# jsh58/Genrich

Measured on AMD Instinct MI355X. Metric: genome bases p-scored/sec, hg38 50M frags, higher is better.
Workload: dtype int32 pileup (1/120 units) + f64 p-values; 1 GPU; hg38 25 contigs (3088286401 bp), 50000000 paired fragments x 1 replicate(s), treatment only, -p 0.01 (BASELINE.json configs[1]); parallelism=chromosome-sharded x1, collectives=none, rccl_nranks=0, intervals=83948696, tables_written_in_step=none: the sweep walks the loose (end, V) slots, p = table p(V)

## Files before the change

genrich_amd/csrc/gx_sbtile.h:

```cpp
#pragma once
#include "gx_sort.h"
#include "gx_tile_fast.h"

namespace gx {

#ifndef GX_EXP_SBT
#define GX_EXP_SBT 0
#endif

constexpr int SBT_NT = 1024;
constexpr int SBT_NW = SBT_NT / 64;
constexpr int SBT_TILES = 1 << SBT_MAXSHIFT;
constexpr int SBT_K = 8;
#ifndef GX_SBT_KP
#define GX_SBT_KP 8
#endif
constexpr int SBT_KP = GX_SBT_KP;
constexpr int SBT_KX = 16;
static_assert(SBT_KX <= 2 * SBT_K && SBT_KP <= SBT_KX, "the slot tables hold 2 x SBT_K x SBT_NW descriptors");
constexpr u32 SBT_SLOT = 256;
constexpr u32 SBT_SLOTS = SBT_K * SBT_NW;
#ifndef GX_SBT_TR
#define GX_SBT_TR 448
#endif
constexpr u32 SBT_PEAK_KEYS = 200;
constexpr u32 SBT_HEAVY = 4096;
constexpr int SBT_MAXR = 8;
constexpr u32 SBT_FCAP = 16384;
constexpr int SBT_TR = GX_SBT_TR;
constexpr int SBT_TR_DENSE = 384;
constexpr int SBT_OCCW = TILE / 32 + 4, SBT_PREW = TILE / 64 + 4;
__host__ __device__ constexpr u32 sbt_tw(u32 tr) { return (u32)(SBT_OCCW + SBT_PREW) + tr + tr / 2; }
constexpr u32 SBT_NOKEY = 0x1000u;
static_assert(SBT_TR % 64 == 0, "the last step of a round reads whole wavefronts of counters");
static_assert((1u << PgCfg<u32>::SHIFT) % SBT_SLOT == 0, "a slot never crosses a page");
static_assert(TILE == 4096, "13-bit LDS keys: 12 bits of offset and the stream");
static_assert((SBT_NW * sbt_tw(64)) % 4 == 0 && (SBT_NW * 96) % 4 == 0, "the scratch is cleared by 16-byte stores (TR: a multiple of 64)");
constexpr u32 SBT_LDS_BYTES = 160u * 1024u - 512u;

struct SbtLds {
  u32 hist[SBT_TILES];
  u32 startC[SBT_TILES + 1];
  int netPref[SBT_TILES];
  u32 cur[2 * SBT_TILES];
  uint4 tinfo[SBT_TILES];
  u32 slotOff[2 * SBT_SLOTS];
  u32 slotCnt[2 * SBT_SLOTS];
  u32 pre[2][2][NXCD + 1];
  u32 lenN[2 * NXCD];
  u32 anyHeavy;
  u32 segN;
  u32 ovfN;
  __attribute__((aligned(8))) u32 scratch[40];
  u32 work;
  u32 overflow;
  u32 rnd[SBT_MAXR + 1];
  u32 nRounds;
  u32 nHeavy;
  uint16_t heavy[SBT_TILES];
  int netW[SBT_TILES];
  u32 vsRed[2];
  __attribute__((aligned(16))) int dyn[4];
};
constexpr u32 SBT_DYN_OFF = (u32)offsetof(SbtLds, dyn);
__host__ __device__ constexpr u32 sbt_keycap(u32 tr) { return ((SBT_LDS_BYTES - SBT_DYN_OFF - SBT_NW * sbt_tw(tr) * 4u) / 2u - 192u) / 64u * 64u; }
constexpr u32 SBT_KEYCAP = sbt_keycap(SBT_TR);
static_assert(sbt_keycap(192) > sbt_keycap(448) && sbt_keycap(448) >= 40960, "the split of the LDS");

constexpr u32 TM_BEDX = 16u;
constexpr u32 TM_BEDIN = 32u;
struct SbtIn {
  PagedStream PS, PE;
  PagedStream PF;
  const u32* sbOffS;
  const u32* sbOffE;
  const u32* sbOffF;
  const u32* tileChrom;
  const DChrom* chroms;
  const int* chromW0;
  u32 nSeg, nTiles;
  int sbShift;
  const FragFix* ff;
  long long* fragAcc;
  BedIn bed;
  u64* fragSum;
};

struct SbtOut {
  TileOut to;
  TileMeta* meta;
  u32* tileSlot;
  u32* hot;
  u32* nBig;
  u32* bigList;
  u32* heavyList;
  u32* nHeavyG;
  u32* ticket;
};

__device__ __forceinline__ void wave_lds_sync() {
  __builtin_amdgcn_fence(__ATOMIC_RELEASE, "wavefront");
  __builtin_amdgcn_wave_barrier();
  __builtin_amdgcn_fence(__ATOMIC_ACQUIRE, "wavefront");
}

__device__ __forceinline__ void st_u32(void* base, u32 index, u32 v) {
  *reinterpret_cast<u32*>(static_cast<char*>(base) + (size_t)(index << 2)) = v;
}

__device__ __forceinline__ u32 sbt_zero() {
  u32 z = 0;
  asm volatile("" : "+s"(z));
  return z;
}

constexpr u32 SBT_NOKEY_F = 0x10000u;
__device__ __forceinline__ int sbt_weight(u32 key) {
  const int w = (int)((0x0C0F14181E283C78ull >> (8 * ((key >> 12) & 7u))) & 0xFFu);
  return (key & 0x8000u) ? -w : w;
}
__device__ __forceinline__ u32 sbt_class_of(int w) {
  u32 c = 8;
#pragma unroll
  for (u32 k = 0; k < 8; k++) c = (int)((0x0C0F14181E283C78ull >> (8 * k)) & 0xFFu) == w ? k : c;
  return c;
}

template <bool FRAC, bool BED>
__device__ __forceinline__ void sbt_tile(const int lane, int* lds, const u32 TR_CAP, const uint16_t* __restrict__ kl, u32 n, u32 t, u32 pos0, u32 len, u32 flags,
                                         int carry, u32 slot, int vsig, const SbtOut& out, u32& bad, bool fragTerms, long long& fhi,
                                         long long& flo, long long& bedExcl) {
  constexpr u32 NOKEY = FRAC ? SBT_NOKEY_F : SBT_NOKEY;
  if (BED && (flags & TM_BEDIN)) {
    long long s = 0;
    for (u32 k = lane; k < n; k += 64) {
      const u32 key = kl[k];
      const int w = FRAC ? sbt_weight(key) : ((key & 0x8000u) ? -GX_UNIT : GX_UNIT);
      s += (long long)w * (long long)(TILE - (key & (TILE - 1)));
    }
    bedExcl += wave_sum(s) + (long long)carry * TILE;
    if (lane == 0) out.to.tileCount[t] = 0;
    return;
  }
  auto offOf = [](u32 key) -> u32 { return FRAC ? (key & (TILE - 1)) | ((key >> 4) & (u32)TILE) : key & (2 * TILE - 1); };
  u32* occ = reinterpret_cast<u32*>(lds);
  u32* pre = reinterpret_cast<u32*>(lds + SBT_OCCW);
  const uint16_t* pre16 = reinterpret_cast<const uint16_t*>(pre);
  int* cnt = lds + SBT_OCCW + SBT_PREW;
  uint16_t* list = reinterpret_cast<uint16_t*>(lds + SBT_OCCW + SBT_PREW + TR_CAP);
  if (!(flags & TM_ACTIVE)) {
    if (lane == 0) out.to.tileCount[t] = 0;
    return;
  }
  constexpr bool active = true;
  const u32 negPos0 = 0u - pos0;
  const bool lastTile = (flags & TM_LAST) != 0;
#ifndef GX_SBT_KR
#define GX_SBT_KR 2
#endif
  constexpr int KR = GX_SBT_KR;
  u32 kr[KR];
#pragma unroll
  for (int q = 0; q < KR; q++) {
    const u32 v = kl[lane + q * 64];
    kr[q] = (u32)lane + q * 64 < n ? v : NOKEY;
  }
  auto mark = [&](u32 key) { const u32 off = offOf(key); atomicOr(&occ[off >> 5], 1u << (off & 31)); };
#pragma unroll
  for (int q = 0; q < KR; q++)
    if (kr[q] != NOKEY) mark(kr[q]);
  for (u32 k = KR * 64 + lane; k < n; k += 64) mark(kl[k]);
  wave_lds_sync();
  const uint2 ww = *reinterpret_cast<const uint2*>(occ + 2 * lane);
  const u32 w0 = ww.x, w1 = ww.y;
  const int c0 = __popc(w0), c = c0 + __popc(w1);
  const int incC = dpp_scan_add(c);
  const u32 exc = (u32)(incC - c);
  const u32 T = (u32)__builtin_amdgcn_readlane(incC, 63);
  pre[lane] = exc | ((exc + (u32)c0) << 16);
  wave_lds_sync();
  int runBase = carry;
  u32 outCount = 0, lastEnd = 0;
  u64 negM = 0, bigM = carry >= FRAG_FAST_MAXV ? ~0ull : 0ull;
  auto rankOf = [&](u32 key) -> u32 {
    const u32 off = offOf(key), wi = off >> 5;
    return (u32)pre16[wi] + (u32)__popc(occ[wi] & ((1u << (off & 31)) - 1u));
  };
  u32 rr[KR];
#pragma unroll
  for (int q = 0; q < KR; q++) rr[q] = rankOf(kr[q]);
  for (u32 r0 = 0; r0 < T; r0 += TR_CAP) {
    if (r0) wave_lds_sync();
    auto put = [&](u32 r, u32 key) {
      r -= r0;
      if (r < (u32)TR_CAP) {
        list[r] = (uint16_t)(key & (TILE - 1));
        atomicAdd(&cnt[r], FRAC ? sbt_weight(key) : ((key & 0x8000u) ? -GX_UNIT : GX_UNIT));
      }
    };
#pragma unroll
    for (int q = 0; q < KR; q++) put(rr[q], kr[q]);
    for (u32 k = KR * 64 + lane; k < n; k += 64) {
      const u32 key = kl[k];
      put(rankOf(key), key);
    }
    wave_lds_sync();
    const u32 nL = min((u32)TR_CAP, T - r0);
    auto loadEl = [&](u32 j, u32& p, int& d120) {
      p = list[j];
      d120 = __hip_atomic_exchange(&cnt[j], 0, __ATOMIC_RELAXED, __HIP_MEMORY_SCOPE_WAVEFRONT);
    };
    auto emit = [&](const u32 p, const int d120, const int incS) {
      const int after = runBase + incS;
      const int before = after - d120;
      const u64 mask = __builtin_amdgcn_uicmp((u32)d120, 0u, 33 ) & __builtin_amdgcn_uicmp(p, negPos0, 33);
      const bool nz = __builtin_amdgcn_inverse_ballot_w64(mask);
      const u32 orank = __builtin_amdgcn_mbcnt_hi((u32)(mask >> 32), __builtin_amdgcn_mbcnt_lo((u32)mask, 0u));
      if (nz) {
        const u32 o = slot + outCount + orank;
        st_u32(out.to.looseEnd, o, pos0 + p);
        st_u32(out.to.looseV, o, (u32)before);
      }
      if (vsig != 0x7FFFFFFF)
        sig_flush_m(out.to.sigMask, slot + outCount, mask & __builtin_amdgcn_sicmp(before, vsig, 39 ), orank, mask);
      if (__builtin_amdgcn_uicmp((u32)after, (u32)FRAG_FAST_MAXV, 35 )) {
        negM |= __ballot(after < 0);
        bigM |= __ballot(after >= FRAG_FAST_MAXV);
      }
      runBase += __builtin_amdgcn_readlane(incS, 63);
      if (FRAC && fragTerms && mask) {
        const u64 below = mask & ((1ull << lane) - 1ull);
        const int prevLane = below ? 63 - __builtin_clzll(below) : 0;
        const u32 pp = (u32)__shfl((int)p, prevLane, 64);
        if (nz && (below || outCount)) frag_term(pos0 + p - (below ? pos0 + pp : lastEnd), before, fhi, flo);
      }
      if (mask) {
        outCount += (u32)__popcll(mask);
        lastEnd = pos0 + (u32)__builtin_amdgcn_readlane((int)p, 63 - __builtin_clzll(mask));
      }
    };
    for (u32 j0 = 0; j0 < nL; j0 += 64) {
      u32 p;
      int d120;
      loadEl(j0 + lane, p, d120);
      emit(p, d120, dpp_scan_add(d120));
    }
  }
  {
    const u32 z = sbt_zero();
    *reinterpret_cast<uint2*>(occ + 2 * lane) = make_uint2(z, z);
  }
  u32 total = 0;
  if (active) {
    total = outCount + (lastTile ? 1u : 0u);
    if (lane == 0) {
      if (lastTile) {
        const u32 o = slot + outCount;
        out.to.looseEnd[o] = len;
        out.to.looseV[o] = runBase;
        if (runBase >= vsig) atomicOr((unsigned long long*)&out.to.sigMask[o >> 6], 1ull << (o & 63));
        if (FRAC && fragTerms && outCount) frag_term(len - lastEnd, runBase, fhi, flo);
        lastEnd = len;
      }
      if (total) out.to.tileLastEnd[t] = lastEnd;
    }
    lastEnd = (u32)__builtin_amdgcn_readfirstlane((int)lastEnd);
    if (negM) bad |= ST_NEG_PILE;
    if (bigM && lane == 0) {
      atomicOr(&out.to.tileDeep[t], 1u);
      if (out.to.ctl) atomicOr(&out.to.ctl->bad, 1u);
    }
  }
  if (lane == 0) out.to.tileCount[t] = total;
  if (total && (vsig != 0x7FFFFFFF || out.to.ctl)) {
    const u32 size = n + 1;
    for (u32 j = total + lane; j < size; j += 64) {
      st_u32(out.to.looseEnd, slot + j, lastEnd);
      st_u32(out.to.looseV, slot + j, 0u);
    }
  }
  wave_lds_sync();
}

template <bool FRAC, bool BED>
__device__ __forceinline__ void sbt_heavy(SbtLds& L, const u32 scrWords, const uint16_t* __restrict__ kl, u32 n, u32 t, u32 pos0, u32 len, u32 flags,
                                          int carry, u32 slot, int vsig, const SbtOut& out, u32& bad, bool fragTerms, const BedIn& bed,
                                          long long& bedExcl) {
  static_assert(SBT_NW * sbt_tw(192) >= TILE, "the counters fit the wavefronts' scratch");
  static_assert(TILE == SBT_NT * 4, "four bases per thread");
  int* cnt = L.dyn;
  const int tid = threadIdx.x;
  const bool active = flags & TM_ACTIVE, lastTile = (flags & TM_LAST) != 0;
  for (u32 i = (u32)tid * 4; i < scrWords; i += SBT_NT * 4) *reinterpret_cast<int4*>(cnt + i) = make_int4(0, 0, 0, 0);
  __syncthreads();
  for (u32 k = tid; k < n; k += SBT_NT) {
    const u32 key = kl[k];
    atomicAdd(&cnt[key & (TILE - 1)], FRAC ? sbt_weight(key) : ((key & 0x8000u) ? -GX_UNIT : GX_UNIT));
  }
  __syncthreads();
  const int4 d4 = *reinterpret_cast<const int4*>(cnt + tid * 4);
  const int d[4] = {d4.x, d4.y, d4.z, d4.w};
  int tot;
  const int ex = block_excl_scan<int, SBT_NT>(d[0] + d[1] + d[2] + d[3], reinterpret_cast<int*>(L.scratch), &tot);
  int run = carry + ex;
  bool nz[4];
  int before[4];
  u32 mine = 0, neg = 0, big = (u32)(tid == 0 && carry >= FRAG_FAST_MAXV);
  const bool bedx = BED && (flags & TM_BEDX) != 0;
  bool save = true, saveEnd = true;
  u32 edgeM = 0;
  if (bedx) {
    const u32 e0 = bed.bedTileOff[t], e1 = bed.bedTileOff[t + 1];
    u32 pre = 0;
    for (u32 i = e0; i < e1; i++) {
      const u32 off = bed.bedEdge[i];
      pre += (u32)(off < (u32)tid * 4);
      if (off - (u32)tid * 4 < 4u) edgeM |= 1u << (off - (u32)tid * 4);
    }
    const bool s0 = bed.tileSave0[t] != 0;
    save = s0 ^ ((pre & 1u) != 0);
    saveEnd = s0 ^ (((e1 - e0) & 1u) != 0);
  }
  long long excl = 0;
#pragma unroll
  for (int j = 0; j < 4; j++) {
    const bool edge = (edgeM >> j) & 1u;
    before[j] = save ? run : V_MARK;
    run += d[j];
    nz[j] = (edge || (save && d[j] != 0)) && active && (pos0 + (u32)tid * 4 + j != 0);
    if (edge) save = !save;
    if (bedx && active && !save && pos0 + (u32)tid * 4 + j < len) excl += run;
    mine += nz[j];
    neg |= (u32)(run < 0);
    big |= (u32)(run >= FRAG_FAST_MAXV);
  }
  if (bedx) bedExcl += wave_sum(excl);
  u32 outCount;
  u32 o = slot + block_excl_scan<u32, SBT_NT>(mine, L.scratch, &outCount);
  u32 lastPos = 0;
#pragma unroll
  for (int j = 0; j < 4; j++)
    if (nz[j]) {
      const u32 p = pos0 + (u32)tid * 4 + j;
      out.to.looseEnd[o] = p;
      out.to.looseV[o] = before[j];
      if (before[j] >= vsig) atomicOr((unsigned long long*)&out.to.sigMask[o >> 6], 1ull << (o & 63));
      lastPos = p;
      o++;
    }
  u32 lastEnd;
  {
    u32 m = lastPos;
#pragma unroll
    for (int dd = 32; dd > 0; dd >>= 1) m = max(m, (u32)__shfl_xor((int)m, dd, 64));
    __syncthreads();
    if (lane_id() == 0) L.scratch[tid >> 6] = m;
    __syncthreads();
    m = 0;
    for (int w = 0; w < SBT_NW; w++) m = max(m, L.scratch[w]);
    lastEnd = m;
    __syncthreads();
  }
  const int endRun = carry + tot;
  u32 total = 0;
  if (active) {
    total = outCount + (lastTile ? 1u : 0u);
    if (tid == 0) {
      if (lastTile) {
        const u32 oc = slot + outCount;
        out.to.looseEnd[oc] = len;
        out.to.looseV[oc] = saveEnd ? endRun : V_MARK;
        if (saveEnd && endRun >= vsig) atomicOr((unsigned long long*)&out.to.sigMask[oc >> 6], 1ull << (oc & 63));
      }
      if (total) out.to.tileLastEnd[t] = lastTile ? len : lastEnd;
    }
    if (lastTile) lastEnd = len;
    if (neg) bad |= ST_NEG_PILE;
    if (__syncthreads_or((int)big) && tid == 0) {
      atomicOr(&out.to.tileDeep[t], 1u);
      if (out.to.ctl) atomicOr(&out.to.ctl->bad, 1u);
    }
  }
  if (tid == 0) out.to.tileCount[t] = total;
  if (FRAC && fragTerms && tid == 0) out.heavyList[atomicAdd(out.nHeavyG, 1u)] = t;
  if (total && (vsig != 0x7FFFFFFF || out.to.ctl))
    for (u32 j = total + tid; j < n + 1; j += SBT_NT) {
      out.to.looseEnd[slot + j] = lastEnd;
      out.to.looseV[slot + j] = 0;
    }
  __syncthreads();
}

__device__ __forceinline__ void sbt_excl_scan2(u32 a, u32 b, uint2* scratch, int tid, u32& exA, u32& exB, u32& totA, u32& totB) {
  const u32 ia = (u32)dpp_scan_add((int)a), ib = (u32)dpp_scan_add((int)b);
  const int w = tid >> 6;
  if ((tid & 63) == 63) scratch[w] = make_uint2(ia, ib);
  __syncthreads();
  if (tid < 64) {
    const uint2 x = tid < SBT_NW ? scratch[tid] : make_uint2(0u, 0u);
    const u32 xa = (u32)dpp_scan_add((int)x.x), xb = (u32)dpp_scan_add((int)x.y);
    if (tid < SBT_NW) scratch[tid] = make_uint2(xa - x.x, xb - x.y);
    if (tid == SBT_NW - 1) scratch[SBT_NW] = make_uint2(xa, xb);
  }
  __syncthreads();
  const uint2 base = scratch[w], tot = scratch[SBT_NW];
  exA = ia - a + base.x;
  exB = ib - b + base.y;
  totA = tot.x;
  totB = tot.y;
  __syncthreads();
}

#ifndef GX_SBT_PREFETCH
#define GX_SBT_PREFETCH 1
#endif
template <bool PAIRS, bool BIG, bool FRAC, int TRC, bool BED>
__device__ __forceinline__ void sbt_bin(const SbtIn& in, const SbtOut& out, u32* __restrict__ st, const u32 segArg, SbtLds& L) {
  static_assert(PAIRS || !BIG, "the second launch exists in pair mode only");
  static_assert(PAIRS || !FRAC, "fractional weights ride pair records only");
  static_assert(!BED || (PAIRS && !FRAC), "-E regions: unit-weight pair records (the tiles with an edge are the second launch's)");
  constexpr u32 LENB = FRAC ? 9u : PAIR_LEN_BITS;
  const bool fragTerms = FRAC && in.fragAcc != nullptr && (u32)__builtin_amdgcn_readfirstlane((int)in.ff->slow) != 0u;
  long long fhi = 0, flo = 0, bedExcl = 0;
  u32 bad = 0;
  constexpr int K = BIG ? 0 : (PAIRS ? SBT_KP : SBT_K);
  constexpr int KX = BIG ? SBT_KX : K;
  constexpr int KR = K ? K : 1;
  constexpr u32 NSLOTS = (u32)KX * SBT_NW;
  constexpr bool OVERLAP = !BIG && GX_SBT_PREFETCH != 0;
  constexpr bool PF = PAIRS && OVERLAP;
  int tid = threadIdx.x, lane = lane_id(), wv = tid >> 6;
  static_assert(TRC % 64 == 0 && TRC >= 192 && TRC <= 448, "touched bases per round");
  constexpr u32 trCap = (u32)TRC;
  constexpr u32 tw = sbt_tw(trCap), scrWords = SBT_NW * tw, keyCap = sbt_keycap(trCap);
  static_assert(tw % 4 == 0, "a wavefront clears its scratch by 16-byte stores");
  int* const scr = L.dyn;
  uint16_t* const keysL = reinterpret_cast<uint16_t*>(L.dyn + scrWords);
  const u32 nSeg = in.nSeg;
  const u32 nT = 1u << in.sbShift;
  const int vsig = (int)__builtin_amdgcn_readfirstlane(loose_vsig(out.to.ctl, !BIG && blockIdx.x == 0 && tid == 0, L.vsRed));
  const uint4* __restrict__ poolS = reinterpret_cast<const uint4*>(in.PS.pool);
  const uint4* __restrict__ poolE = reinterpret_cast<const uint4*>(in.PE.pool);
  constexpr bool hasBed = BED;
#ifndef GX_SBT_FREG
#define GX_SBT_FREG 1
#endif
  u32 seg = 0, segTileBase = 0, par = 0;
  u32 ci = 0;
  uint4 kS[KR], kE[PAIRS ? 1 : KR];
  u32 segN = 0, ciN = 0, lenRegN = 0;
  bool haveN = false;
  uint4 kN[PF ? KR : 1];
  u32 tk = 0;
  bool drawn = false;
  int stage = 0;
#pragma unroll
  for (int i = 0; i < (PF ? KR : 1); i++) kN[i] = make_uint4(0u, 0u, 0u, 0u);
  auto clearOwn = [&]() {
    int* mine = scr + (u32)__builtin_amdgcn_readfirstlane(wv) * tw;
    const int z = (int)sbt_zero();
    for (u32 i = (u32)lane * 4; i < tw; i += 64 * 4) *reinterpret_cast<int4*>(mine + i) = make_int4(z, z, z, z);
    wave_lds_sync();
    if (lane == 0) mine[SBT_OCCW + TILE / 64] = -1;
  };
  auto askLens = [&](u32 sg) {
    lenRegN = 0;
    if (sg < nSeg && tid < 2 * NXCD) {
      const u32 li = (u32)(tid & (NXCD - 1)) * nSeg + sg;
      if (PAIRS)
        lenRegN = tid < NXCD ? list_len<u32>(in.PS, li) : list_len<u64>(in.PF, li);
      else
        lenRegN = list_len<u32>(tid < NXCD ? in.PS : in.PE, li);
    }
  };
  auto askChrom = [&]() {
    haveN = segN < nSeg;
    ciN = 0;
    if (haveN && tid < (int)nT) {
      const u32 t = (segN << in.sbShift) + (u32)tid;
      if (t < in.nTiles) ciN = in.tileChrom[t];
    }
  };
  auto stashChrom = [&]() {
    if (tid < (int)nT) L.cur[tid] = ciN;
  };
  auto lensToLds = [&]() {
    if (wv != 0) return;
    if (tid < 2 * NXCD) L.lenN[tid] = lenRegN;
    if (tid == 0) L.ovfN = 0;
    wave_lds_sync();
    if (tid < 2) {
      u32 a = 0, ns = 0;
      for (int x = 0; x < NXCD; x++) {
        L.pre[par ^ 1u][tid][x] = a;
        const u32 l = L.lenN[tid * NXCD + x];
        a += l;
        ns += (l + SBT_SLOT - 1) / SBT_SLOT;
      }
      L.pre[par ^ 1u][tid][NXCD] = a;
      if (ns > NSLOTS && (tid == 0 || !PAIRS)) L.ovfN = 1;
    }
  };
  auto descOwn = [&](u32 sg, u32 pr) {
    constexpr int ND = (PAIRS ? 1 : 2) * KX;
    static_assert(ND <= 64, "a lane per slot of the wavefront");
    if (lane < ND) {
      const int q = lane / KX;
      const u32 k = (u32)(lane % KX) * SBT_NW + (u32)wv;
      const PagedStream& P = q ? in.PE : in.PS;
      const u32* pre = L.pre[pr][q];
      u32 x = NXCD, k0 = 0, acc = 0;
      for (u32 y = 0; y < NXCD; y++) {
        const u32 ns = (pre[y + 1] - pre[y] + SBT_SLOT - 1) / SBT_SLOT;
        if (x == NXCD && k < acc + ns) {
          x = y;
          k0 = acc;
        }
        acc += ns;
      }
      u32 ptr = 0;
      u32 cnt = 0;
      if (x < NXCD) {
        const u32 off = (k - k0) * SBT_SLOT;
        const u32 jp = off >> PgCfg<u32>::SHIFT, li = x * nSeg + sg;
        const u32 page = jp ? P.pt[(size_t)li * P.jmax + jp] - 1u : first_page(li);
        ptr = (page << PgCfg<u32>::SHIFT) + (off & ((1u << PgCfg<u32>::SHIFT) - 1u));
        cnt = min(SBT_SLOT, pre[x + 1] - pre[x] - off);
      }
      L.slotOff[(u32)q * NSLOTS + k] = ptr;
      L.slotCnt[(u32)q * NSLOTS + k] = cnt;
    }
    wave_lds_sync();
  };
  auto loadRecs = [&](bool have, u32 sg, u32 pr, uint4 (&dS)[KR], uint4 (&dE)[PAIRS ? 1 : KR]) {
    const bool ov = !have || L.ovfN != 0;
    const u32 z = PF ? sbt_zero() : 0u;
#pragma unroll
    for (int i = 0; i < K; i++) {
      const u32 c = ov ? 0u : (u32)__builtin_amdgcn_readfirstlane((int)L.slotCnt[i * SBT_NW + wv]);
      dS[i] = make_uint4(z, z, z, z);
      if ((u32)lane * 4 < c) dS[i] = poolS[(L.slotOff[i * SBT_NW + wv] >> 2) + lane];
    }
#pragma unroll
    for (int i = 0; i < (PAIRS ? 1 : K); i++) {
      const u32 c = ov || PAIRS ? 0u : (u32)__builtin_amdgcn_readfirstlane((int)L.slotCnt[NSLOTS + i * SBT_NW + wv]);
      dE[i] = make_uint4(z, z, z, z);
      if (!PAIRS && (u32)lane * 4 < c) dE[i] = poolE[(L.slotOff[NSLOTS + i * SBT_NW + wv] >> 2) + lane];
    }
  };
  auto finishNext = [&]() {
    if (stage < 1) {
      if (wv == 0) {
        if (!drawn && tid == 0) tk = atomicAdd(out.ticket, 1u);
        const u32 sN = (u32)__builtin_amdgcn_readfirstlane((int)tk);
        askLens(sN);
        if (tid == 0) L.segN = sN;
      }
      __syncthreads();
      segN = L.segN;
      askChrom();
    }
    if (GX_EXP_SBT == 4 || GX_EXP_SBT == 5) stashChrom();
    if (GX_EXP_SBT == 4) return;
    if (stage < 2) lensToLds();
    if (GX_EXP_SBT == 5) return;
    if (stage < 3) {
      __syncthreads();
      if constexpr (PF)
      {
        if (haveN) descOwn(segN, par ^ 1u);
        loadRecs(haveN, segN, par ^ 1u, kN, kE);
      }
      stashChrom();
    }
  };
  auto rotate = [&]() {
    seg = segN;
    segTileBase = seg << in.sbShift;
    if constexpr (!BIG) ci = tid < (int)nT ? L.cur[tid] : 0u;
    else ci = ciN;
    par ^= 1u;
    if constexpr (PF) {
#pragma unroll
      for (int i = 0; i < K; i++) kS[i] = kN[i];
    }
  };
  auto bin = [&]() {
  if constexpr (!BIG) {
    asm volatile("" : "+v"(tid));
    lane = tid & 63;
    wv = tid >> 6;
  }
  if (OVERLAP && tid == 0) tk = atomicAdd(out.ticket, 1u);
  drawn = OVERLAP;
  auto loadTi = [&]() {
    uint4 ti = make_uint4(0u, 0u, 0u, 0u);
    if (tid < (int)nT) {
      const u32 t = segTileBase + tid;
      if (t < in.nTiles) {
        const DChrom c = in.chroms[ci];
        const u32 tl = t - c.tileBase;
        ti.x = tl << TB;
        ti.y = c.len;
        ti.z = (chrom_active(c) ? TM_ACTIVE : 0u) | (tl + 1 == c.nTiles ? TM_LAST : 0u);
        ti.w = (u32)in.chromW0[ci];
      }
    }
    return ti;
  };
  u32 bedBefore = 0, bedMine = 0;
  bool bedInside = false;
  auto loadBed = [&](const uint4& ti) {
    if (hasBed && tid < (int)nT && segTileBase + tid < in.nTiles) {
      const u32 t = segTileBase + tid;
      bedBefore = in.bed.bedTileOff[t];
      bedMine = in.bed.bedTileOff[t + 1] - bedBefore;
      const bool s0 = in.bed.tileSave0[t] != 0;
      bedInside = !bedMine && !s0 && !(ti.z & TM_LAST);
      if (bedInside && (ti.z & TM_ACTIVE)) return TM_BEDIN;
      if (bedMine || (!s0 && (ti.z & TM_LAST))) return TM_BEDX;
    }
    return 0u;
  };
  auto expLeave = [&]() {
    if (tid < (int)nT && segTileBase + tid < in.nTiles) {
      const u32 t = segTileBase + tid;
      TileMeta m{};
      m.slot = t;
      out.meta[t] = m;
      out.tileSlot[t] = t;
      if (t + 1 == in.nTiles) out.tileSlot[in.nTiles] = in.nTiles;
      out.to.tileCount[t] = 0;
    }
  };
  if (GX_EXP_SBT == 4) { expLeave(); return; }
  if constexpr (!PF) {
    descOwn(seg, par);
    loadRecs(true, seg, par, kS, kE);
  }
  uint4 ti = loadTi();
  const u32 bedx = loadBed(ti);
  const bool ovfSlots = L.ovfN != 0;
  u32 cS[KR], cE[PAIRS ? 1 : KR];
#pragma unroll
  for (int i = 0; i < K; i++)
    cS[i] = ovfSlots ? 0u : (u32)__builtin_amdgcn_readfirstlane((int)L.slotCnt[i * SBT_NW + wv]);
#pragma unroll
  for (int i = 0; i < (PAIRS ? 1 : K); i++)
    cE[i] = ovfSlots || PAIRS ? 0u : (u32)__builtin_amdgcn_readfirstlane((int)L.slotCnt[NSLOTS + i * SBT_NW + wv]);
  const BinSrc<u64> srcF{reinterpret_cast<const u64*>(in.PF.pool), in.PF.pt, nSeg, in.PF.jmax, seg, L.pre[par][1]};
  const u32 nF = PAIRS && !ovfSlots ? L.pre[par][1][NXCD] : 0u;
  u64 fReg = 0;
  if (GX_SBT_FREG && PAIRS && (u32)tid < nF) fReg = srcF.at((u32)tid);
  auto singleAt = [&](u32 i) -> u64 { return GX_SBT_FREG && i == (u32)tid ? fReg : srcF.at(i); };
  if (tid < SBT_TILES) {
    L.hist[tid] = 0;
    if (FRAC) L.netW[tid] = 0;
  }
  if (tid == 0) {
    L.overflow = ovfSlots || (PAIRS && (nF > SBT_FCAP || L.pre[par][0][NXCD] + nF > 65535u)) ? 1u : 0u;
    L.nHeavy = 0;
    L.nRounds = 0;
    L.anyHeavy = 0;
  }
  __syncthreads();
  if (GX_EXP_SBT == 5) { expLeave(); return; }
  if (GX_EXP_SBT == 1) {
    u32 x = 0;
#pragma unroll
    for (int i = 0; i < K; i++) x ^= kS[i].x ^ kS[i].y ^ kS[i].z ^ kS[i].w ^ kE[PAIRS ? 0 : i].x;
    if (x == 0xDEADBEEFu) atomicOr(st, 1u << 30);
  }
  auto keyAt = [](const uint4& v, int j) -> u32 { return j == 0 ? v.x : j == 1 ? v.y : j == 2 ? v.z : v.w; };
  auto slotsFrom = [&](int i0, auto&& f) {
    for (int i = i0; i < KX; i += 4) {
      u32 c[4];
      uint4 v[4];
#pragma unroll
      for (int q = 0; q < 4; q++) {
        c[q] = i + q < KX ? (u32)__builtin_amdgcn_readfirstlane((int)L.slotCnt[(i + q) * SBT_NW + wv]) : 0u;
        v[q] = make_uint4(0u, 0u, 0u, 0u);
        if ((u32)lane * 4 < c[q]) v[q] = poolS[(L.slotOff[(i + q) * SBT_NW + wv] >> 2) + lane];
      }
#pragma unroll
      for (int q = 0; q < 4; q++) {
        if (!c[q]) continue;
#pragma unroll
        for (int j = 0; j < 4; j++)
          if ((u32)lane * 4 + j < c[q]) f(keyAt(v[q], j));
      }
    }
  };
  auto pairTs = [](u32 r) -> u32 { return r >> (PAIR_LEN_BITS + TB); };
  auto pairEnd = [](u32 r) -> u32 { return (r >> PAIR_LEN_BITS) + (r & ((1u << LENB) - 1u)); };
  auto pairCls = [](u32 r) -> u32 { return FRAC ? ((r >> 9) & 7u) << 12 : 0u; };
  auto fCls = [](u64 r) -> u32 {
    const int w = (int)(int8_t)(r & 0xFF);
    return FRAC ? (sbt_class_of(w < 0 ? -w : w) & 7u) << 12 : 0u;
  };
  auto histPair = [&](u32 r) {
    const u32 ts = pairTs(r), te = pairEnd(r) >> TB;
    atomicAdd(&L.hist[ts], ts == te ? 65537u : 1u);
    if (ts != te) {
      atomicAdd(&L.hist[te], 65536u);
      if (FRAC) {
        const int w = sbt_weight(pairCls(r));
        atomicAdd(&L.netW[ts], w);
        atomicAdd(&L.netW[te], -w);
      }
    }
  };
  if (PAIRS) {
#pragma unroll
    for (int i = 0; i < K; i++) {
      if (cS[i] == SBT_SLOT) {
#pragma unroll
        for (int j = 0; j < 4; j++) histPair(keyAt(kS[i], j));
      } else if (cS[i]) {
#pragma unroll
        for (int j = 0; j < 4; j++)
          if ((u32)lane * 4 + j < cS[i]) histPair(keyAt(kS[i], j));
      }
    }
    if (!ovfSlots) slotsFrom(K, [&](u32 r) { histPair(r); });
    if (nF <= SBT_FCAP)
      for (u32 i = tid; i < nF; i += SBT_NT) {
        const u64 r = singleAt(i);
        const int w = (int)(int8_t)(r & 0xFF);
        const bool ok = FRAC ? sbt_class_of(w < 0 ? -w : w) < 8u : (w == GX_UNIT || w == -GX_UNIT);
        if (ok) {
          atomicAdd(&L.hist[(u32)(r >> 32) - segTileBase], w > 0 ? 1u : 65536u);
          if (FRAC) atomicAdd(&L.netW[(u32)(r >> 32) - segTileBase], w);
        } else
          L.overflow = 2;
      }
  } else if constexpr (!PAIRS) {
  if (GX_EXP_SBT != 1)
#pragma unroll
  for (int i = 0; i < SBT_K; i++) {
    if (cS[i] == SBT_SLOT) {
#pragma unroll
      for (int j = 0; j < 4; j++) atomicAdd(&L.hist[(keyAt(kS[i], j) >> TB) - segTileBase], 1u);
    } else if (cS[i]) {
#pragma unroll
      for (int j = 0; j < 4; j++)
        if ((u32)lane * 4 + j < cS[i]) atomicAdd(&L.hist[(keyAt(kS[i], j) >> TB) - segTileBase], 1u);
    }
    if (cE[i] == SBT_SLOT) {
#pragma unroll
      for (int j = 0; j < 4; j++) atomicAdd(&L.hist[(keyAt(kE[i], j) >> TB) - segTileBase], 65536u);
    } else if (cE[i]) {
#pragma unroll
      for (int j = 0; j < 4; j++)
        if ((u32)lane * 4 + j < cE[i]) atomicAdd(&L.hist[(keyAt(kE[i], j) >> TB) - segTileBase], 65536u);
    }
  }
  }
  if (OVERLAP && wv == 0) {
    const u32 sN = (u32)__builtin_amdgcn_readfirstlane((int)tk);
    askLens(sN);
    if (tid == 0) L.segN = sN;
  }
  __syncthreads();
  if constexpr (OVERLAP) {
    segN = L.segN;
    askChrom();
    stage = 1;
  }
  {
    u32 h = tid < (int)nT ? L.hist[tid] : 0u;
    const u32 nS = h & 0xFFFFu, nE = h >> 16;
    u32 totK, totN;
    u32 exK, exN;
    sbt_excl_scan2(nS + nE, (u32)(FRAC ? (tid < (int)nT ? L.netW[tid] : 0) : (int)nS - (int)nE), reinterpret_cast<uint2*>(L.scratch), tid, exK, exN,
                   totK, totN);
    if (tid < (int)nT) {
      L.startC[tid] = exK;
      L.netPref[tid] = (int)exN;
    }
    if (tid == 0) L.startC[nT] = totK;
    if (PAIRS && !BIG && (nS + nE > SBT_HEAVY || (bedx & TM_BEDX))) L.anyHeavy = 1;
  }
  __syncthreads();
  if constexpr (PAIRS && !BIG) {
    const bool big = L.anyHeavy != 0 || ovfSlots || L.startC[nT] > keyCap || L.overflow == 1;
    if (big) {
      if (tid == 0) out.bigList[atomicAdd(out.nBig, 1u)] = seg;
      return;
    }
  }
  if (BIG && tid == 0) {
    u32 nr = 0;
    bool fits = true;
    if (L.startC[nT] <= keyCap) {
      L.rnd[0] = 0;
      L.rnd[1] = nT;
      nr = 1;
    } else if (!ovfSlots) {
      u32 tb = 0;
      L.rnd[0] = 0;
      while (tb < nT && fits) {
        u32 lo = tb, hi = nT;
        const u32 lim = L.startC[tb] + keyCap;
        while (lo < hi) {
          const u32 mid = (lo + hi + 1) >> 1;
          if (L.startC[mid] <= lim) lo = mid; else hi = mid - 1;
        }
        const u32 te = lo;
        if (te == tb || nr == (u32)SBT_MAXR) fits = false;
        else {
          L.rnd[++nr] = te;
          tb = te;
        }
      }
    }
    L.nRounds = fits ? nr : 0u;
  }
  if (BIG) __syncthreads();
  const u32 nRounds = BIG ? L.nRounds : 1u;
  const u32 ovfWord = PAIRS ? L.overflow : 0u;
  const bool ovfReal = ovfSlots || (BIG ? nRounds == 0 : L.startC[nT] > keyCap) || ovfWord != 0;
  const bool ovf = ovfReal || GX_EXP_SBT == 1 || GX_EXP_SBT == 2;
  if (ovfReal && tid == 0) atomicOr(st, ovfWord == 2 ? ST_SB_FRAC : ST_SB_FULL);
  if (!PAIRS && seg == 0 && tid == 0 && in.sbOffF[nSeg] != 0) atomicOr(st, ST_SB_FRAC);
  const u32 segS = in.sbOffS[seg], segE = in.sbOffE[seg];
  const u32 segSlot = PAIRS ? segS + segTileBase : segS + segE + segTileBase;
  const int segNet = PAIRS ? (int)segE : GX_UNIT * ((int)segS - (int)segE);
  if (tid < (int)nT) {
    const u32 t = segTileBase + tid;
    const u32 h = ovf ? 0u : L.hist[tid];
    const u32 nS = h & 0xFFFFu, nE = h >> 16;
    const u32 sc = ovf ? 0u : L.startC[tid];
    L.cur[tid] = sc;
    L.cur[SBT_TILES + tid] = sc + nS;
    if (nS >= HOT16 / GX_UNIT || nE >= HOT16 / GX_UNIT) atomicOr(out.hot, 1u);
    if (t < in.nTiles) {
      TileMeta m;
      m.sb = 0; m.eb = 0; m.fb = 0;
      m.nS = nS; m.nE = nE; m.nF = 0;
      m.carry = ovf ? 0 : segNet + (FRAC ? 1 : GX_UNIT) * L.netPref[tid] - (int)ti.w;
      m.ci = 0;
      m.pos0 = ti.x; m.len = ti.y; m.flags = ti.z;
      m.slot = segSlot + sc + (u32)tid + bedBefore;
      out.meta[t] = m;
      L.tinfo[tid] = make_uint4(ti.x, ti.y, ((bedInside ? ti.z & ~TM_ACTIVE : ti.z) | bedx) | ((nS + nE) << 8), (u32)m.carry);
      static_assert((TM_BEDX | TM_BEDIN) < 256u, "the tile's flags take the low byte, its key count the rest");
      if (hasBed) L.netPref[tid] = (int)bedBefore;
      out.tileSlot[t] = m.slot;
      if (t + 1 == in.nTiles) out.tileSlot[in.nTiles] = m.slot + nS + nE + 1 + bedMine;
    }
  }
  if constexpr (PAIRS && !BIG) {
    if (tid < (int)nT && !ovf) {
      const u32 hA = L.hist[tid];
      const u32 nk = (hA & 0xFFFFu) + (hA >> 16);
      const u32 pos = nk > SBT_PEAK_KEYS ? atomicAdd(&L.nHeavy, 1u) : nT - 1u - atomicAdd(&L.nRounds, 1u);
      L.heavy[pos] = (uint16_t)tid;
    }
  }
  if (ovf) {
    if (tid < (int)nT && segTileBase + tid < in.nTiles) out.to.tileCount[segTileBase + tid] = 0;
    return;
  }
  if (tid == 0) L.work = 0;
  __syncthreads();
  auto place = [&](u32 key, u32 curBase, u32 flag) {
    keysL[atomicAdd(&L.cur[curBase + (key >> TB) - segTileBase], 1u)] = (uint16_t)((key & (TILE - 1)) | flag);
  };
  auto tiles = [&](u32 tileEnd, u32 keyBase) {
    for (;;) {
      u32 b = 0;
      if (lane == 0) b = atomicAdd(&L.work, 1u);
      b = (u32)__builtin_amdgcn_readfirstlane((int)b);
      if (b >= tileEnd) break;
      if constexpr (PAIRS && !BIG) b = (u32)__builtin_amdgcn_readfirstlane((int)L.heavy[b]);
      const u32 t = segTileBase + b;
      if (t >= in.nTiles) continue;
      const uint4 tf = L.tinfo[b];
      const u32 sc = L.startC[b];
      const u32 fz = (u32)__builtin_amdgcn_readfirstlane((int)tf.z), n = fz >> 8;
      if (BIG && !(BED && (fz & TM_BEDIN)) && (n > SBT_HEAVY || (BED && (fz & TM_BEDX)))) {
        if (lane == 0) L.heavy[atomicAdd(&L.nHeavy, 1u)] = (uint16_t)b;
        continue;
      }
      const u32 bedSlots = hasBed ? (u32)__builtin_amdgcn_readfirstlane(L.netPref[b]) : 0u;
      sbt_tile<FRAC, BED>(lane, scr + (u32)__builtin_amdgcn_readfirstlane(wv) * tw, trCap, keysL + (sc - keyBase), n, t, tf.x, tf.y, fz & 0xFFu, (int)tf.w,
                     segSlot + sc + b + bedSlots, vsig, out, bad, fragTerms, fhi, flo, bedExcl);
    }
    if constexpr (BIG) {
    __syncthreads();
    const u32 nH = L.nHeavy;
    if (nH) {
      for (u32 i = 0; i < nH; i++) {
        const u32 b = L.heavy[i], t = segTileBase + b;
        const uint4 tf = L.tinfo[b];
        const u32 sc = L.startC[b], n = tf.z >> 8;
        sbt_heavy<FRAC, BED>(L, scrWords, keysL + (sc - keyBase), n, t, tf.x, tf.y, tf.z & 0xFFu, (int)tf.w,
                        segSlot + sc + b + (hasBed ? (u32)L.netPref[b] : 0u), vsig, out, bad, fragTerms, in.bed, bedExcl);
      }
      for (u32 i = (u32)tid * 4; i < scrWords; i += SBT_NT * 4) *reinterpret_cast<int4*>(scr + i) = make_int4(0, 0, 0, 0);
      __syncthreads();
      if (tid < SBT_NW) scr[(u32)tid * tw + SBT_OCCW + TILE / 64] = -1;
      if (tid == 0) L.nHeavy = 0;
      __syncthreads();
    }
    }
  };
  if constexpr (PAIRS && !BIG) {
    {
      auto placePair = [&](u32 r) {
        const u32 e = pairEnd(r), ts = pairTs(r), te = e >> TB;
        const u32 so = ((r >> PAIR_LEN_BITS) & (TILE - 1)) | pairCls(r), eo = (e & (TILE - 1)) | 0x8000u | pairCls(r);
        const u32 ps = atomicAdd(&L.cur[ts], ts == te ? 2u : 1u);
        const u32 pe = ts == te ? ps + 1u : atomicAdd(&L.cur[te], 1u);
        keysL[ps] = (uint16_t)so;
        keysL[pe] = (uint16_t)eo;
      };
#pragma unroll
      for (int i = 0; i < K; i++) {
        if (cS[i] == SBT_SLOT) {
#pragma unroll
          for (int j = 0; j < 4; j++) placePair(keyAt(kS[i], j));
        } else if (cS[i]) {
#pragma unroll
          for (int j = 0; j < 4; j++)
            if ((u32)lane * 4 + j < cS[i]) placePair(keyAt(kS[i], j));
        }
      }
      for (u32 i = tid; i < nF; i += SBT_NT) {
        const u64 r = singleAt(i);
        const u32 off = (u32)(r >> 8) & (TILE - 1);
        keysL[atomicAdd(&L.cur[(u32)(r >> 32) - segTileBase], 1u)] = (uint16_t)(off | ((r & 0x80) ? 0x8000u : 0u) | fCls(r));
      }
      if constexpr (OVERLAP) {
        lensToLds();
        stage = 2;
      }
      __syncthreads();
      if (GX_EXP_SBT == 3) {
        if (tid < (int)nT && segTileBase + tid < in.nTiles) out.to.tileCount[segTileBase + tid] = keysL[L.startC[tid]] == 0xFFFFu;
        return;
      }
      if constexpr (PF) {
        if (haveN) descOwn(segN, par ^ 1u);
        loadRecs(haveN, segN, par ^ 1u, kN, kE);
        stashChrom();
        stage = 3;
      }
      tiles(nT, 0u);
      clearOwn();
    }
  } else if constexpr (BIG) {
    {
      for (u32 round = 0; round < nRounds; round++) {
        const u32 tileBeg = L.rnd[round], tileEnd = L.rnd[round + 1], keyBase = L.startC[tileBeg];
        if (round) {
          __syncthreads();
          if (tid == 0) L.work = tileBeg;
          __syncthreads();
        }
        slotsFrom(0, [&](u32 r) {
          const u32 e = pairEnd(r), ts = pairTs(r), te = e >> TB;
          if (ts - tileBeg < tileEnd - tileBeg) keysL[atomicAdd(&L.cur[ts], 1u) - keyBase] = (uint16_t)(((r >> PAIR_LEN_BITS) & (TILE - 1)) | pairCls(r));
          if (te - tileBeg < tileEnd - tileBeg) keysL[atomicAdd(&L.cur[te], 1u) - keyBase] = (uint16_t)((e & (TILE - 1)) | 0x8000u | pairCls(r));
        });
        for (u32 i = tid; i < nF; i += SBT_NT) {
          const u64 r = singleAt(i);
          const u32 tl = (u32)(r >> 32) - segTileBase, off = (u32)(r >> 8) & (TILE - 1);
          if (tl - tileBeg < tileEnd - tileBeg) keysL[atomicAdd(&L.cur[tl], 1u) - keyBase] = (uint16_t)(off | ((r & 0x80) ? 0x8000u : 0u) | fCls(r));
        }
        __syncthreads();
        tiles(tileEnd, keyBase);
      }
    }
  } else {
#pragma unroll
  for (int i = 0; i < SBT_K; i++) {
    if (cS[i] == SBT_SLOT) {
      u32 ps[4];
#pragma unroll
      for (int j = 0; j < 4; j++) ps[j] = atomicAdd(&L.cur[(keyAt(kS[i], j) >> TB) - segTileBase], 1u);
#pragma unroll
      for (int j = 0; j < 4; j++) keysL[ps[j]] = (uint16_t)(keyAt(kS[i], j) & (TILE - 1));
    } else if (cS[i]) {
#pragma unroll
      for (int j = 0; j < 4; j++)
        if ((u32)lane * 4 + j < cS[i]) place(keyAt(kS[i], j), 0u, 0u);
    }
    if (cE[i] == SBT_SLOT) {
      u32 ps[4];
#pragma unroll
      for (int j = 0; j < 4; j++) ps[j] = atomicAdd(&L.cur[SBT_TILES + (keyAt(kE[i], j) >> TB) - segTileBase], 1u);
#pragma unroll
      for (int j = 0; j < 4; j++) keysL[ps[j]] = (uint16_t)((keyAt(kE[i], j) & (TILE - 1)) | 0x8000u);
    } else if (cE[i]) {
#pragma unroll
      for (int j = 0; j < 4; j++)
        if ((u32)lane * 4 + j < cE[i]) place(keyAt(kE[i], j), (u32)SBT_TILES, 0x8000u);
    }
  }
  if constexpr (OVERLAP) {
    lensToLds();
    stage = 2;
  }
  __syncthreads();
  if (GX_EXP_SBT == 3) {
    if (tid < (int)nT && segTileBase + tid < in.nTiles) out.to.tileCount[segTileBase + tid] = keysL[L.startC[tid]] == 0xFFFFu;
    return;
  }
  tiles(nT, 0u);
  clearOwn();
  }
  };
  clearOwn();
  if constexpr (BIG) {
    askLens(segArg);
    segN = segArg;
    askChrom();
    lensToLds();
    __syncthreads();
    rotate();
    bin();
  } else {
    finishNext();
    for (;;) {
      __syncthreads();
      rotate();
      if (seg >= nSeg) break;
      stage = 0;
      bin();
      finishNext();
    }
  }
  if (FRAC && fragTerms) {
    fhi = wave_sum(fhi);
    flo = wave_sum(flo);
    if (lane == 0) {
      if (fhi) atomicAdd((u64*)&in.fragAcc[0], (u64)fhi);
      if (flo) atomicAdd((u64*)&in.fragAcc[1], (u64)flo);
    }
  }
  if (bedExcl && lane == 0) atomicAdd(&in.fragSum[((BIG ? segArg : blockIdx.x) * SBT_NW + (u32)wv) % FRAG_SLOTS], (u64)(-(bedExcl / GX_UNIT)));
  if (bad && lane == 0) atomicOr(st, bad);
}

template <bool PAIRS, bool BIG, bool FRAC, int TRC = SBT_TR, bool BED = false>
__global__ __launch_bounds__(SBT_NT) void k_sbtile(SbtIn in, SbtOut out, u32* __restrict__ st) {
  extern __shared__ __attribute__((aligned(16))) unsigned char sbt_raw[];
  SbtLds& L = *reinterpret_cast<SbtLds*>(sbt_raw);
  if constexpr (!BIG)
    sbt_bin<PAIRS, false, FRAC, TRC, BED>(in, out, st, 0u, L);
  else {
    const u32 nBig = out.bigList ? *out.nBig : in.nSeg;
    for (u32 item = blockIdx.x; item < nBig; item += gridDim.x) {
      sbt_bin<PAIRS, true, FRAC, TRC, BED>(in, out, st, out.bigList ? out.bigList[item] : item, L);
      __syncthreads();
    }
  }
}

}
```

Before: 2782 Gbases/s.

## Process pairs of light adjacent tiles together in one wavefront

Result: faster. 2865 Gbases/s, median of 6 (+3.0%).

```diff
diff --git a/genrich_amd/csrc/gx_sbtile.h b/genrich_amd/csrc/gx_sbtile.h
--- a/genrich_amd/csrc/gx_sbtile.h
+++ b/genrich_amd/csrc/gx_sbtile.h
@@ -126,6 +126,76 @@
   return c;
 }
 
+template <bool FRAC>
+struct SbtRun {
+  const u32 pos0, negPos0, slot;
+  const int vsig;
+  int runBase;
+  u32 outCount = 0, lastEnd = 0;
+  u64 negM = 0, bigM;
+  __device__ __forceinline__ SbtRun(u32 pos0_, int carry, u32 slot_, int vsig_)
+      : pos0(pos0_), negPos0(0u - pos0_), slot(slot_), vsig(vsig_), runBase(carry), bigM(carry >= FRAG_FAST_MAXV ? ~0ull : 0ull) {}
+  __device__ __forceinline__ void emit(const int lane, const SbtOut& out, bool fragTerms, long long& fhi, long long& flo, const u32 p, const int d120,
+                                       const int incS) {
+    const int after = runBase + incS;
+    const int before = after - d120;
+    const u64 mask = __builtin_amdgcn_uicmp((u32)d120, 0u, 33 ) & __builtin_amdgcn_uicmp(p, negPos0, 33);
+    const bool nz = __builtin_amdgcn_inverse_ballot_w64(mask);
+    const u32 orank = __builtin_amdgcn_mbcnt_hi((u32)(mask >> 32), __builtin_amdgcn_mbcnt_lo((u32)mask, 0u));
+    if (nz) {
+      const u32 o = slot + outCount + orank;
+      st_u32(out.to.looseEnd, o, pos0 + p);
+      st_u32(out.to.looseV, o, (u32)before);
+    }
+    if (vsig != 0x7FFFFFFF)
+      sig_flush_m(out.to.sigMask, slot + outCount, mask & __builtin_amdgcn_sicmp(before, vsig, 39 ), orank, mask);
+    if (__builtin_amdgcn_uicmp((u32)after, (u32)FRAG_FAST_MAXV, 35 )) {
+      negM |= __ballot(after < 0);
+      bigM |= __ballot(after >= FRAG_FAST_MAXV);
+    }
+    runBase += __builtin_amdgcn_readlane(incS, 63);
+    if (FRAC && fragTerms && mask) {
+      const u64 below = mask & ((1ull << lane) - 1ull);
+      const int prevLane = below ? 63 - __builtin_clzll(below) : 0;
+      const u32 pp = (u32)__shfl((int)p, prevLane, 64);
+      if (nz && (below || outCount)) frag_term(pos0 + p - (below ? pos0 + pp : lastEnd), before, fhi, flo);
+    }
+    if (mask) {
+      outCount += (u32)__popcll(mask);
+      lastEnd = pos0 + (u32)__builtin_amdgcn_readlane((int)p, 63 - __builtin_clzll(mask));
+    }
+  }
+  __device__ __forceinline__ void finish(const int lane, const SbtOut& out, u32 t, u32 n, u32 len, bool lastTile, u32& bad, bool fragTerms,
+                                         long long& fhi, long long& flo) {
+    const u32 total = outCount + (lastTile ? 1u : 0u);
+    if (lane == 0) {
+      if (lastTile) {
+        const u32 o = slot + outCount;
+        out.to.looseEnd[o] = len;
+        out.to.looseV[o] = runBase;
+        if (runBase >= vsig) atomicOr((unsigned long long*)&out.to.sigMask[o >> 6], 1ull << (o & 63));
+        if (FRAC && fragTerms && outCount) frag_term(len - lastEnd, runBase, fhi, flo);
+        lastEnd = len;
+      }
+      if (total) out.to.tileLastEnd[t] = lastEnd;
+    }
+    lastEnd = (u32)__builtin_amdgcn_readfirstlane((int)lastEnd);
+    if (negM) bad |= ST_NEG_PILE;
+    if (bigM && lane == 0) {
+      atomicOr(&out.to.tileDeep[t], 1u);
+      if (out.to.ctl) atomicOr(&out.to.ctl->bad, 1u);
+    }
+    if (lane == 0) out.to.tileCount[t] = total;
+    if (total && (vsig != 0x7FFFFFFF || out.to.ctl)) {
+      const u32 size = n + 1;
+      for (u32 j = total + lane; j < size; j += 64) {
+        st_u32(out.to.looseEnd, slot + j, lastEnd);
+        st_u32(out.to.looseV, slot + j, 0u);
+      }
+    }
+  }
+};
+
 template <bool FRAC, bool BED>
 __device__ __forceinline__ void sbt_tile(const int lane, int* lds, const u32 TR_CAP, const uint16_t* __restrict__ kl, u32 n, u32 t, u32 pos0, u32 len, u32 flags,
                                          int carry, u32 slot, int vsig, const SbtOut& out, u32& bad, bool fragTerms, long long& fhi,
@@ -152,8 +222,6 @@
     if (lane == 0) out.to.tileCount[t] = 0;
     return;
   }
-  constexpr bool active = true;
-  const u32 negPos0 = 0u - pos0;
   const bool lastTile = (flags & TM_LAST) != 0;
 #ifndef GX_SBT_KR
 #define GX_SBT_KR 2
@@ -179,9 +247,7 @@
   const u32 T = (u32)__builtin_amdgcn_readlane(incC, 63);
   pre[lane] = exc | ((exc + (u32)c0) << 16);
   wave_lds_sync();
-  int runBase = carry;
-  u32 outCount = 0, lastEnd = 0;
-  u64 negM = 0, bigM = carry >= FRAG_FAST_MAXV ? ~0ull : 0ull;
+  SbtRun<FRAC> run(pos0, carry, slot, vsig);
   auto rankOf = [&](u32 key) -> u32 {
     const u32 off = offOf(key), wi = off >> 5;
     return (u32)pre16[wi] + (u32)__popc(occ[wi] & ((1u << (off & 31)) - 1u));
@@ -210,75 +276,103 @@
       p = list[j];
       d120 = __hip_atomic_exchange(&cnt[j], 0, __ATOMIC_RELAXED, __HIP_MEMORY_SCOPE_WAVEFRONT);
     };
-    auto emit = [&](const u32 p, const int d120, const int incS) {
-      const int after = runBase + incS;
-      const int before = after - d120;
-      const u64 mask = __builtin_amdgcn_uicmp((u32)d120, 0u, 33 ) & __builtin_amdgcn_uicmp(p, negPos0, 33);
-      const bool nz = __builtin_amdgcn_inverse_ballot_w64(mask);
-      const u32 orank = __builtin_amdgcn_mbcnt_hi((u32)(mask >> 32), __builtin_amdgcn_mbcnt_lo((u32)mask, 0u));
-      if (nz) {
-        const u32 o = slot + outCount + orank;
-        st_u32(out.to.looseEnd, o, pos0 + p);
-        st_u32(out.to.looseV, o, (u32)before);
-      }
-      if (vsig != 0x7FFFFFFF)
-        sig_flush_m(out.to.sigMask, slot + outCount, mask & __builtin_amdgcn_sicmp(before, vsig, 39 ), orank, mask);
-      if (__builtin_amdgcn_uicmp((u32)after, (u32)FRAG_FAST_MAXV, 35 )) {
-        negM |= __ballot(after < 0);
-        bigM |= __ballot(after >= FRAG_FAST_MAXV);
-      }
-      runBase += __builtin_amdgcn_readlane(incS, 63);
-      if (FRAC && fragTerms && mask) {
-        const u64 below = mask & ((1ull << lane) - 1ull);
-        const int prevLane = below ? 63 - __builtin_clzll(below) : 0;
-        const u32 pp = (u32)__shfl((int)p, prevLane, 64);
-        if (nz && (below || outCount)) frag_term(pos0 + p - (below ? pos0 + pp : lastEnd), before, fhi, flo);
-      }
-      if (mask) {
-        outCount += (u32)__popcll(mask);
-        lastEnd = pos0 + (u32)__builtin_amdgcn_readlane((int)p, 63 - __builtin_clzll(mask));
-      }
-    };
     for (u32 j0 = 0; j0 < nL; j0 += 64) {
       u32 p;
       int d120;
       loadEl(j0 + lane, p, d120);
-      emit(p, d120, dpp_scan_add(d120));
+      run.emit(lane, out, fragTerms, fhi, flo, p, d120, dpp_scan_add(d120));
     }
   }
   {
     const u32 z = sbt_zero();
     *reinterpret_cast<uint2*>(occ + 2 * lane) = make_uint2(z, z);
   }
-  u32 total = 0;
-  if (active) {
-    total = outCount + (lastTile ? 1u : 0u);
-    if (lane == 0) {
-      if (lastTile) {
-        const u32 o = slot + outCount;
-        out.to.looseEnd[o] = len;
-        out.to.looseV[o] = runBase;
-        if (runBase >= vsig) atomicOr((unsigned long long*)&out.to.sigMask[o >> 6], 1ull << (o & 63));
-        if (FRAC && fragTerms && outCount) frag_term(len - lastEnd, runBase, fhi, flo);
-        lastEnd = len;
-      }
-      if (total) out.to.tileLastEnd[t] = lastEnd;
-    }
-    lastEnd = (u32)__builtin_amdgcn_readfirstlane((int)lastEnd);
-    if (negM) bad |= ST_NEG_PILE;
-    if (bigM && lane == 0) {
-      atomicOr(&out.to.tileDeep[t], 1u);
-      if (out.to.ctl) atomicOr(&out.to.ctl->bad, 1u);
-    }
-  }
-  if (lane == 0) out.to.tileCount[t] = total;
-  if (total && (vsig != 0x7FFFFFFF || out.to.ctl)) {
-    const u32 size = n + 1;
-    for (u32 j = total + lane; j < size; j += 64) {
-      st_u32(out.to.looseEnd, slot + j, lastEnd);
-      st_u32(out.to.looseV, slot + j, 0u);
-    }
-  }
+  run.finish(lane, out, t, n, len, lastTile, bad, fragTerms, fhi, flo);
+  wave_lds_sync();
+}
+
+#ifndef GX_SBT_X2
+#define GX_SBT_X2 1
+#endif
+constexpr u32 SBT_X2_KEYS = GX_SBT_KR * 64;
+constexpr int SBT_X2_CNT = SBT_OCCW + SBT_PREW;
+constexpr int SBT_X2_OCC_B = SBT_X2_CNT + (int)SBT_X2_KEYS;
+constexpr int SBT_X2_CNT_B = SBT_X2_OCC_B + SBT_OCCW;
+constexpr int SBT_X2_LIST = SBT_X2_CNT + SBT_TR;
+constexpr int SBT_X2_LIST_B = SBT_X2_LIST + (int)SBT_X2_KEYS / 2;
+constexpr int SBT_X2_PRE_B = SBT_X2_LIST_B + (int)SBT_X2_KEYS / 2;
+constexpr bool SBT_X2_FITS = SBT_X2_CNT_B + (int)SBT_X2_KEYS <= SBT_X2_LIST && SBT_X2_PRE_B + SBT_PREW <= (int)sbt_tw(SBT_TR);
+static_assert(SBT_TR != 448 || GX_SBT_KR != 2 || SBT_X2_FITS, "the pair layout fits a wavefront's scratch: sbt_tw(SBT_TR)");
+static_assert(SBT_X2_OCC_B % 2 == 0, "a lane reads its two bitmap words as one 8-byte word");
+
+__device__ __forceinline__ void sbt_tile_x2(const int lane, int* lds, const uint16_t* __restrict__ klA, const u32 nA, const u32 nB, const u32 t,
+                                            const uint4 tfA, const uint4 tfB, const u32 slotA, const int vsig, const SbtOut& out, u32& bad) {
+  constexpr int KR = GX_SBT_KR;
+  u32* occA = reinterpret_cast<u32*>(lds);
+  u32* occB = reinterpret_cast<u32*>(lds + SBT_X2_OCC_B);
+  u32* preA = reinterpret_cast<u32*>(lds + SBT_OCCW);
+  u32* preB = reinterpret_cast<u32*>(lds + SBT_X2_PRE_B);
+  int* cntA = lds + SBT_X2_CNT;
+  int* cntB = lds + SBT_X2_CNT_B;
+  uint16_t* listA = reinterpret_cast<uint16_t*>(lds + SBT_X2_LIST);
+  uint16_t* listB = reinterpret_cast<uint16_t*>(lds + SBT_X2_LIST_B);
+  const uint16_t* __restrict__ klB = klA + nA;
+  u32 ka[KR], kb[KR];
+#pragma unroll
+  for (int q = 0; q < KR; q++) {
+    const u32 va = klA[lane + q * 64], vb = klB[lane + q * 64];
+    ka[q] = (u32)lane + q * 64 < nA ? va : SBT_NOKEY;
+    kb[q] = (u32)lane + q * 64 < nB ? vb : SBT_NOKEY;
+  }
+  if (lane == 0) preB[TILE / 64] = ~0u;
+  auto mark = [](u32* occ, u32 key) { const u32 off = key & (2 * TILE - 1); atomicOr(&occ[off >> 5], 1u << (off & 31)); };
+#pragma unroll
+  for (int q = 0; q < KR; q++) {
+    if (ka[q] != SBT_NOKEY) mark(occA, ka[q]);
+    if (kb[q] != SBT_NOKEY) mark(occB, kb[q]);
+  }
+  wave_lds_sync();
+  const uint2 wa = *reinterpret_cast<const uint2*>(occA + 2 * lane), wb = *reinterpret_cast<const uint2*>(occB + 2 * lane);
+  const int ca0 = __popc(wa.x), ca = ca0 + __popc(wa.y), cb0 = __popc(wb.x), cb = cb0 + __popc(wb.y);
+  const int incA = dpp_scan_add(ca), incB = dpp_scan_add(cb);
+  const u32 excA = (u32)(incA - ca), excB = (u32)(incB - cb);
+  const u32 TA = (u32)__builtin_amdgcn_readlane(incA, 63), TB = (u32)__builtin_amdgcn_readlane(incB, 63);
+  preA[lane] = excA | ((excA + (u32)ca0) << 16);
+  preB[lane] = excB | ((excB + (u32)cb0) << 16);
+  wave_lds_sync();
+  auto put = [](const u32* occ, const u32* pre, int* cnt, uint16_t* list, u32 key) {
+    const u32 off = key & (2 * TILE - 1), wi = off >> 5;
+    const u32 r = (u32)reinterpret_cast<const uint16_t*>(pre)[wi] + (u32)__popc(occ[wi] & ((1u << (off & 31)) - 1u));
+    if (r < SBT_X2_KEYS) {
+      list[r] = (uint16_t)(key & (TILE - 1));
+      atomicAdd(&cnt[r], (key & 0x8000u) ? -GX_UNIT : GX_UNIT);
+    }
+  };
+#pragma unroll
+  for (int q = 0; q < KR; q++) {
+    put(occA, preA, cntA, listA, ka[q]);
+    put(occB, preB, cntB, listB, kb[q]);
+  }
+  wave_lds_sync();
+  SbtRun<false> runA(tfA.x, (int)tfA.w, slotA, vsig), runB(tfB.x, (int)tfB.w, slotA + nA + 1u, vsig);
+  long long f0 = 0, f1 = 0;
+  auto step = [&](u32 j) {
+    const u32 pA = listA[j], pB = listB[j];
+    const int dA = __hip_atomic_exchange(&cntA[j], 0, __ATOMIC_RELAXED, __HIP_MEMORY_SCOPE_WAVEFRONT);
+    const int dB = __hip_atomic_exchange(&cntB[j], 0, __ATOMIC_RELAXED, __HIP_MEMORY_SCOPE_WAVEFRONT);
+    const int sA = dpp_scan_add(dA), sB = dpp_scan_add(dB);
+    runA.emit(lane, out, false, f0, f1, pA, dA, sA);
+    runB.emit(lane, out, false, f0, f1, pB, dB, sB);
+  };
+  step((u32)lane);
+  if (max(TA, TB) > 64u) step(64u + (u32)lane);
+  {
+    const u32 z = sbt_zero();
+    *reinterpret_cast<uint2*>(occA + 2 * lane) = make_uint2(z, z);
+    *reinterpret_cast<uint2*>(occB + 2 * lane) = make_uint2(z, z);
+  }
+  runA.finish(lane, out, t, nA, tfA.y, (tfA.z & TM_LAST) != 0, bad, false, f0, f1);
+  runB.finish(lane, out, t + 1u, nB, tfB.y, (tfB.z & TM_LAST) != 0, bad, false, f0, f1);
   wave_lds_sync();
 }
 
@@ -429,6 +523,7 @@
   constexpr u32 NSLOTS = (u32)KX * SBT_NW;
   constexpr bool OVERLAP = !BIG && GX_SBT_PREFETCH != 0;
   constexpr bool PF = PAIRS && OVERLAP;
+  constexpr bool X2 = GX_SBT_X2 != 0 && SBT_X2_FITS && PAIRS && !BIG && !FRAC && !BED && TRC == SBT_TR;
   int tid = threadIdx.x, lane = lane_id(), wv = tid >> 6;
   static_assert(TRC % 64 == 0 && TRC >= 192 && TRC <= 448, "touched bases per round");
   constexpr u32 trCap = (u32)TRC;
@@ -851,11 +946,17 @@
     }
   }
   if constexpr (PAIRS && !BIG) {
-    if (tid < (int)nT && !ovf) {
-      const u32 hA = L.hist[tid];
-      const u32 nk = (hA & 0xFFFFu) + (hA >> 16);
+    const u32 hA = tid < (int)nT && !ovf ? L.hist[tid] : 0u;
+    const u32 nk = (hA & 0xFFFFu) + (hA >> 16);
+    bool paired = false;
+    if constexpr (X2) {
+      const bool can = tid < (int)nT && segTileBase + (u32)tid < in.nTiles && (ti.z & TM_ACTIVE) && nk <= SBT_X2_KEYS;
+      const int canN = __shfl_xor((int)can, 1, 64);
+      paired = can && canN != 0;
+    }
+    if (tid < (int)nT && !ovf && !(paired && (tid & 1))) {
       const u32 pos = nk > SBT_PEAK_KEYS ? atomicAdd(&L.nHeavy, 1u) : nT - 1u - atomicAdd(&L.nRounds, 1u);
-      L.heavy[pos] = (uint16_t)tid;
+      L.heavy[pos] = (uint16_t)((u32)tid | (paired ? 0x8000u : 0u));
     }
   }
   if (ovf) {
@@ -868,12 +969,29 @@
     keysL[atomicAdd(&L.cur[curBase + (key >> TB) - segTileBase], 1u)] = (uint16_t)((key & (TILE - 1)) | flag);
   };
   auto tiles = [&](u32 tileEnd, u32 keyBase) {
+    u32 nFront = 0, gap = 0;
+    if constexpr (X2) {
+      nFront = (u32)__builtin_amdgcn_readfirstlane((int)L.nHeavy);
+      gap = tileEnd - nFront - (u32)__builtin_amdgcn_readfirstlane((int)L.nRounds);
+      tileEnd -= gap;
+    }
     for (;;) {
       u32 b = 0;
       if (lane == 0) b = atomicAdd(&L.work, 1u);
       b = (u32)__builtin_amdgcn_readfirstlane((int)b);
       if (b >= tileEnd) break;
-      if constexpr (PAIRS && !BIG) b = (u32)__builtin_amdgcn_readfirstlane((int)L.heavy[b]);
+      if constexpr (PAIRS && !BIG) b = (u32)__builtin_amdgcn_readfirstlane((int)L.heavy[b < nFront ? b : b + gap]);
+      if constexpr (X2) {
+        if (b & 0x8000u) {
+          b &= 0x7FFFu;
+          const uint4 tfA = L.tinfo[b], tfB = L.tinfo[b + 1u];
+          const u32 sc = L.startC[b];
+          const u32 nA = (u32)__builtin_amdgcn_readfirstlane((int)tfA.z) >> 8, nB = (u32)__builtin_amdgcn_readfirstlane((int)tfB.z) >> 8;
+          sbt_tile_x2(lane, scr + (u32)__builtin_amdgcn_readfirstlane(wv) * tw, keysL + (sc - keyBase), nA, nB, segTileBase + b, tfA, tfB,
+                      segSlot + sc + b, vsig, out, bad);
+          continue;
+        }
+      }
       const u32 t = segTileBase + b;
       if (t >= in.nTiles) continue;
       const uint4 tf = L.tinfo[b];
```
